# nicoloalbergoni/DeepLabV3Plus-Augmented-SuperResolution

Hardware: AMD Instinct MI355X
Metric: augmented-copies/sec (fwd+realign+SR-iter) @512x512 (higher is better)
Workload: dtype f32 (pointwise GEMMs: operands split into f16 hi+lo, hi*hi+hi*lo+lo*hi on f16 MFMA, f32 accumulate)

## Files before the change

### deeplabv3plus-augmented-superresolution_amd/csrc/sepconv.hip

```cpp
#include "asr_common.h"

#ifndef ASR_SEPCONV_PACKED_SPLIT
#define ASR_SEPCONV_PACKED_SPLIT 1
#endif

typedef float f32x4 __attribute__((ext_vector_type(4)));
typedef float f32x16 __attribute__((ext_vector_type(16)));
typedef _Float16 f16x4 __attribute__((ext_vector_type(4)));
typedef _Float16 f16x8 __attribute__((ext_vector_type(8)));

namespace {

constexpr int SF_TH = 8, SF_TW = 14, SF_VALID = SF_TH * SF_TW, SF_M = 128, SF_N = 128;

template <int CTRL>
__device__ __forceinline__ f32x4 sf_dpp4(f32x4 v) {
    f32x4 r;
#pragma unroll
    for (int i = 0; i < 4; ++i) {
        const float f = v[i];
        r[i] = __int_as_float(__builtin_amdgcn_mov_dpp(__float_as_int(f), CTRL, 0xF, 0xF, true));
    }
    return r;
}

__device__ __forceinline__ int sf_swz(int slot, int line) { return (slot & ~15) | ((slot ^ line) & 15); }

#ifdef ASR_DIAG_SEPCONV_MAX_VGPR
#define ASR_SEPCONV_ATTR __attribute__((amdgpu_num_vgpr(ASR_DIAG_SEPCONV_MAX_VGPR)))
#else
#define ASR_SEPCONV_ATTR
#endif
template <int CIN>
__global__ __launch_bounds__(512) ASR_PK_F32 ASR_SEPCONV_ATTR void sepconv_fused_kernel(const float* __restrict__ x, const float* __restrict__ wd,
                                                            const float* __restrict__ bd, const _Float16* __restrict__ wp,
                                                            const float* __restrict__ bp, float* __restrict__ y, int batch, int h,
                                                            int w, int ldx, int ldy, int npad, int pre_relu, int dw_relu,
                                                            int out_relu) {
#if ASR_SEPCONV_PACKED_SPLIT
    asr_enable_f16_saturation();
#endif
#ifdef ASR_DIAG_SEPCONV_TOP_VGPR
    ASR_DIAG_TOUCH_VGPR(ASR_DIAG_SEPCONV_TOP_VGPR);
#endif
    constexpr int QUADS = CIN / 4;
    constexpr int HALVES = 32 / QUADS;
    constexpr int RPT = SF_TH / HALVES;
    constexpr int LB = CIN * 4;
    constexpr int OCTS = CIN / 8;
    constexpr int A_BYTES = SF_M * LB, B_BYTES = OCTS * SF_N * 16;
    extern __shared__ __attribute__((aligned(16))) char sf_lds[];
    char* const A = sf_lds;
    char* const Bh = sf_lds + A_BYTES;
    char* const Bl = Bh + B_BYTES;
    const int tid = threadIdx.x, lane = tid & 63, wave = tid >> 6, l32 = lane & 31, hh = lane >> 5;
    typedef unsigned int u32x4 __attribute__((ext_vector_type(4)));
    {
        const long long plane = (long long)CIN * npad;
        for (int i = tid; i < OCTS * SF_N; i += 512) {
            const int oct = i >> 7, col = i & 127;
            const _Float16* src = wp + ((long long)oct * npad + col) * 8;
            *reinterpret_cast<u32x4*>(Bh + i * 16) = *reinterpret_cast<const u32x4*>(src);
            *reinterpret_cast<u32x4*>(Bl + i * 16) = *reinterpret_cast<const u32x4*>(src + plane);
        }
    }
    const int lane16 = lane & 15, slot = wave * 4 + (lane >> 4);
    const int q = slot % QUADS, ry0 = (slot / QUADS) * RPT, ch = q * 4;
    f32x4 wk[9];
#pragma unroll
    for (int t = 0; t < 9; ++t) wk[t] = *reinterpret_cast<const f32x4*>(wd + t * CIN + ch);
    const f32x4 bv = *reinterpret_cast<const f32x4*>(bd + ch);
    const f32x4 zero = {0.f, 0.f, 0.f, 0.f};
    const int wm = wave & 3, wn = wave >> 2;
    const float bp0 = bp[wn * 64 + l32], bp1 = bp[wn * 64 + 32 + l32];

    const int tiles_x = (w + SF_TW - 1) / SF_TW, tiles_y = (h + SF_TH - 1) / SF_TH;
    const long long total = (long long)batch * tiles_y * tiles_x;
    f32x4 in[RPT + 2];
    auto request_rows = [&](long long t) {
        const int tx0 = (int)(t % tiles_x) * SF_TW;
        const long long tt = t / tiles_x;
        const int ty0 = (int)(tt % tiles_y) * SF_TH;
        const float* xin = x + (tt / tiles_y) * h * w * ldx + ch;
        const int ixc = min(max(tx0 - 1 + lane16, 0), w - 1);
#pragma unroll
        for (int r = 0; r < RPT + 2; ++r) {
            const int iy = min(max(ty0 + ry0 - 1 + r, 0), h - 1);
            in[r] = *reinterpret_cast<const f32x4*>(xin + ((long long)iy * w + ixc) * ldx);
        }
    };
    const long long per_wg = (total + gridDim.x - 1) / gridDim.x;
    const long long first = (long long)blockIdx.x * per_wg, last = min(first + per_wg, total);
    if (first < last) request_rows(first);
    for (long long tile = first; tile < last; ++tile) {
        const int x0 = (int)(tile % tiles_x) * SF_TW;
        const long long tt = tile / tiles_x;
        const int y0 = (int)(tt % tiles_y) * SF_TH;
        const long long b = tt / tiles_y;
        __syncthreads();
        const int ix = x0 - 1 + lane16;
        const bool col_ok = ix >= 0 && ix < w;
        f32x4 win[3][3];
#pragma unroll
        for (int r = 0; r < RPT + 2; ++r) {
            const int iy = y0 + ry0 - 1 + r;
            f32x4 c = in[r];
            if (pre_relu) {
#pragma unroll
                for (int i = 0; i < 4; ++i) c[i] = fmaxf(c[i], 0.f);
            }
            c = (col_ok && iy >= 0 && iy < h) ? c : zero;
            win[2][1] = c;
            win[2][0] = sf_dpp4<0x111>(c);
            win[2][2] = sf_dpp4<0x101>(c);
            if (r >= 2) {
                f32x4 acc = bv;
#pragma unroll
                for (int ky = 0; ky < 3; ++ky)
#pragma unroll
                    for (int kx = 0; kx < 3; ++kx) acc += win[ky][kx] * wk[ky * 3 + kx];
                if (dw_relu) {
#pragma unroll
                    for (int i = 0; i < 4; ++i) acc[i] = fmaxf(acc[i], 0.f);
                }
                typedef unsigned int u32x2 __attribute__((ext_vector_type(2)));
#if ASR_SEPCONV_PACKED_SPLIT
                unsigned int h01, h23, l01, l23;
                asr_split4_f16_saturating_mode(acc[0], acc[1], acc[2], acc[3], h01, h23, l01, l23);
                u32x2 h2 = {h01, h23}, l2 = {l01, l23};
#else
                f16x4 hi, lo;
#pragma unroll
                for (int i = 0; i < 4; ++i) {
                    _Float16 hf, lf;
                    asr_split_f16(acc[i], hf, lf);
                    hi[i] = hf;
                    lo[i] = lf;
                }
                u32x2 h2 = __builtin_bit_cast(u32x2, hi), l2 = __builtin_bit_cast(u32x2, lo);
#endif
                {
                    const auto sx = __builtin_amdgcn_permlane16_swap(h2.x, l2.x, false, false);
                    const auto sy = __builtin_amdgcn_permlane16_swap(h2.y, l2.y, false, false);
                    h2.x = sx[0]; l2.x = sx[1];
                    h2.y = sy[0]; l2.y = sy[1];
                }
                const u32x4 out = {h2.x, h2.y, l2.x, l2.y};
                if (lane16 >= 1 && lane16 <= SF_TW) {
                    const int line = (ry0 + r - 2) * SF_TW + lane16 - 1;
                    *reinterpret_cast<u32x4*>(A + line * LB + sf_swz(((q & 1) ? OCTS : 0) + (q >> 1), line) * 16) = out;
                }
            }
#pragma unroll
            for (int k = 0; k < 3; ++k) {
                win[0][k] = win[1][k];
                win[1][k] = win[2][k];
            }
        }
        request_rows(min(tile + 1, last - 1));
        __syncthreads();
        f32x16 acc2[2];
#pragma unroll
        for (int j = 0; j < 2; ++j)
#pragma unroll
            for (int e = 0; e < 16; ++e) acc2[j][e] = 0.0f;
        const int m = wm * 32 + l32;
        const char* const aline = A + m * LB;
#pragma unroll
        for (int kk = 0; kk < CIN / 16; ++kk) {
            const int oct = 2 * kk + hh;
            const f16x8 ah = *reinterpret_cast<const f16x8*>(aline + sf_swz(oct, m) * 16);
            const f16x8 al = *reinterpret_cast<const f16x8*>(aline + sf_swz(OCTS + oct, m) * 16);
#pragma unroll
            for (int j = 0; j < 2; ++j) {
                const int col = wn * 64 + j * 32 + l32;
                const f16x8 bh = *reinterpret_cast<const f16x8*>(Bh + (oct * SF_N + col) * 16);
                const f16x8 bl = *reinterpret_cast<const f16x8*>(Bl + (oct * SF_N + col) * 16);
                acc2[j] = __builtin_amdgcn_mfma_f32_32x32x16_f16(al, bh, acc2[j], 0, 0, 0);
                acc2[j] = __builtin_amdgcn_mfma_f32_32x32x16_f16(ah, bl, acc2[j], 0, 0, 0);
                acc2[j] = __builtin_amdgcn_mfma_f32_32x32x16_f16(ah, bh, acc2[j], 0, 0, 0);
            }
        }
        float* const ybase = y + (b * h * w) * ldy + wn * 64 + l32;
#pragma unroll
        for (int e = 0; e < 16; ++e) {
            const int line = wm * 32 + (e & 3) + 8 * (e >> 2) + 4 * hh;
            const int ty = line / SF_TW, tx = line - ty * SF_TW;
            const int oy = y0 + ty, ox = x0 + tx;
            if (line < SF_VALID && oy < h && ox < w) {
                float* const o = ybase + ((long long)oy * w + ox) * ldy;
                float v0 = acc2[0][e] + bp0, v1 = acc2[1][e] + bp1;
                if (out_relu) { v0 = fmaxf(v0, 0.f); v1 = fmaxf(v1, 0.f); }
                o[0] = v0;
                o[32] = v1;
            }
        }
    }
}

template <int CIN>
int launch_sepconv_fused(const float* x, const float* wd, const float* bd, const void* wp, const float* bp, float* y, int batch,
                         int h, int w, int ldx, int ldy, int npad, int pre_relu, int dw_relu, int out_relu, hipStream_t s) {
    constexpr int lds = SF_M * CIN * 4 + 2 * (CIN / 8) * SF_N * 16;
    const int cus = asr_device_cu_count();
    ASR_REQUIRE(cus > 0, "asr_sepconv_fused_f16x3: cannot query the device");
    static AsrDeviceOnce once;
    ASR_HIP_CHECK(asr_allow_dynamic_lds(once, reinterpret_cast<const void*>(sepconv_fused_kernel<CIN>), lds));
    const long long tiles = (long long)batch * asr_cdiv(h, SF_TH) * asr_cdiv(w, SF_TW);
    const long long want = (long long)cus * (lds <= 80 * 1024 ? 2 : 1);
    const int grid = (int)(tiles < want ? tiles : want);
    hipLaunchKernelGGL(sepconv_fused_kernel<CIN>, dim3(grid), dim3(512), lds, s, x, wd, bd, reinterpret_cast<const _Float16*>(wp), bp, y,
                       batch, h, w, ldx, ldy, npad, pre_relu, dw_relu, out_relu);
    ASR_LAUNCH_CHECK();
    return ASR_OK;
}

}

extern "C" int asr_sepconv_fused_f16x3(const float* x, const float* w_dw, const float* bias_dw, const void* w_pw_packed,
                                       const float* bias_pw, float* y, int batch, int h, int w, int cin, int cout, int ldx,
                                       int ldy, int pre_relu, int dw_relu, int out_relu, asr_stream_t stream) {
    ASR_REQUIRE(x && w_dw && bias_dw && w_pw_packed && bias_pw && y, "asr_sepconv_fused_f16x3: null pointer");
    ASR_REQUIRE(batch > 0 && h > 0 && w > 0 && ldx >= cin && ldy >= cout, "asr_sepconv_fused_f16x3: bad geometry");
    ASR_UNSUPPORTED(!((cin == 64 || cin == 128) && cout == 128),
                    "asr_sepconv_fused_f16x3: cin in {64, 128} -> 128 only (got %d -> %d)", cin, cout);
    ASR_UNSUPPORTED((ldx & 3) || ((reinterpret_cast<uintptr_t>(x) | reinterpret_cast<uintptr_t>(w_dw) |
                                   reinterpret_cast<uintptr_t>(bias_dw) | reinterpret_cast<uintptr_t>(w_pw_packed)) & 15),
                    "asr_sepconv_fused_f16x3: ldx %% 4 == 0 and 16-byte aligned x / weights required");
    ASR_UNSUPPORTED((long long)h * w * ldx > 0x7fffffffLL, "asr_sepconv_fused_f16x3: image too large");
    hipStream_t s = asr_stream(stream);
    const int npad = 128;
    if (cin == 64)
        return launch_sepconv_fused<64>(x, w_dw, bias_dw, w_pw_packed, bias_pw, y, batch, h, w, ldx, ldy, npad, pre_relu, dw_relu, out_relu, s);
    return launch_sepconv_fused<128>(x, w_dw, bias_dw, w_pw_packed, bias_pw, y, batch, h, w, ldx, ldy, npad, pre_relu, dw_relu, out_relu, s);
}
```

Measured before the change: 2174.

## Walk vertical strips per workgroup and carry halo rows between steps

Result: no change. 2187, median of 6 (+0.6%).

```diff
diff --git a/deeplabv3plus-augmented-superresolution_amd/csrc/sepconv.hip b/deeplabv3plus-augmented-superresolution_amd/csrc/sepconv.hip
--- a/deeplabv3plus-augmented-superresolution_amd/csrc/sepconv.hip
+++ b/deeplabv3plus-augmented-superresolution_amd/csrc/sepconv.hip
@@ -53,6 +53,8 @@
     char* const A = sf_lds;
     char* const Bh = sf_lds + A_BYTES;
     char* const Bl = Bh + B_BYTES;
+    float* const bias2 = reinterpret_cast<float*>(A + SF_VALID * LB);
+    static_assert((SF_M - SF_VALID) * LB >= SF_N * 4, "the spare LDS lines hold the pointwise bias");
     const int tid = threadIdx.x, lane = tid & 63, wave = tid >> 6, l32 = lane & 31, hh = lane >> 5;
     typedef unsigned int u32x4 __attribute__((ext_vector_type(4)));
     {
@@ -72,38 +74,48 @@
     const f32x4 bv = *reinterpret_cast<const f32x4*>(bd + ch);
     const f32x4 zero = {0.f, 0.f, 0.f, 0.f};
     const int wm = wave & 3, wn = wave >> 2;
-    const float bp0 = bp[wn * 64 + l32], bp1 = bp[wn * 64 + 32 + l32];
-
-    const int tiles_x = (w + SF_TW - 1) / SF_TW, tiles_y = (h + SF_TH - 1) / SF_TH;
-    const long long total = (long long)batch * tiles_y * tiles_x;
+    if (tid < SF_N) bias2[tid] = bp[tid];
+
+    const int strips_x = (w + SF_TW - 1) / SF_TW;
+    const int steps = ((h + RPT - 1) / RPT + HALVES - 1) / HALVES;
+    const int hoff = HALVES > 1 ? steps * RPT : 0;
+    const int rbase = HALVES > 1 ? (ry0 ? hoff : 0) : 0;
+    const long long total = (long long)batch * strips_x * steps;
     f32x4 in[RPT + 2];
-    auto request_rows = [&](long long t) {
-        const int tx0 = (int)(t % tiles_x) * SF_TW;
-        const long long tt = t / tiles_x;
-        const int ty0 = (int)(tt % tiles_y) * SF_TH;
-        const float* xin = x + (tt / tiles_y) * h * w * ldx + ch;
-        const int ixc = min(max(tx0 - 1 + lane16, 0), w - 1);
-#pragma unroll
-        for (int r = 0; r < RPT + 2; ++r) {
-            const int iy = min(max(ty0 + ry0 - 1 + r, 0), h - 1);
+    auto request_rows = [&](long long b, int sx, int st, bool carry) {
+        const float* xin = x + b * h * w * ldx + ch;
+        const int ixc = min(max(sx * SF_TW - 1 + lane16, 0), w - 1);
+        const int yb = st * RPT + rbase - 1;
+        if (carry) {
+            in[0] = in[RPT];
+            in[1] = in[RPT + 1];
+        } else {
+#pragma unroll
+            for (int r = 0; r < 2; ++r) {
+                const int iy = min(max(yb + r, 0), h - 1);
+                in[r] = *reinterpret_cast<const f32x4*>(xin + ((long long)iy * w + ixc) * ldx);
+            }
+        }
+#pragma unroll
+        for (int r = 2; r < RPT + 2; ++r) {
+            const int iy = min(max(yb + r, 0), h - 1);
             in[r] = *reinterpret_cast<const f32x4*>(xin + ((long long)iy * w + ixc) * ldx);
         }
     };
     const long long per_wg = (total + gridDim.x - 1) / gridDim.x;
     const long long first = (long long)blockIdx.x * per_wg, last = min(first + per_wg, total);
-    if (first < last) request_rows(first);
-    for (long long tile = first; tile < last; ++tile) {
-        const int x0 = (int)(tile % tiles_x) * SF_TW;
-        const long long tt = tile / tiles_x;
-        const int y0 = (int)(tt % tiles_y) * SF_TH;
-        const long long b = tt / tiles_y;
+    int st = (int)(first % steps), sx = (int)((first / steps) % strips_x);
+    long long b = first / steps / strips_x;
+    if (first < last) request_rows(b, sx, st, false);
+    for (long long u = first; u < last; ++u) {
+        const int x0 = sx * SF_TW, y0 = st * RPT;
         __syncthreads();
         const int ix = x0 - 1 + lane16;
         const bool col_ok = ix >= 0 && ix < w;
         f32x4 win[3][3];
 #pragma unroll
         for (int r = 0; r < RPT + 2; ++r) {
-            const int iy = y0 + ry0 - 1 + r;
+            const int iy = y0 + rbase - 1 + r;
             f32x4 c = in[r];
             if (pre_relu) {
 #pragma unroll
@@ -157,7 +169,17 @@
                 win[1][k] = win[2][k];
             }
         }
-        request_rows(min(tile + 1, last - 1));
+        int nst = st + 1, nsx = sx;
+        long long nb = b;
+        if (nst == steps) {
+            nst = 0;
+            if (++nsx == strips_x) {
+                nsx = 0;
+                ++nb;
+            }
+        }
+        const bool more = u + 1 < last;
+        request_rows(more ? nb : b, more ? nsx : sx, more ? nst : st, more && nst != 0);
         __syncthreads();
         f32x16 acc2[2];
 #pragma unroll
@@ -181,12 +203,13 @@
                 acc2[j] = __builtin_amdgcn_mfma_f32_32x32x16_f16(ah, bh, acc2[j], 0, 0, 0);
             }
         }
+        const float bp0 = bias2[wn * 64 + l32], bp1 = bias2[wn * 64 + 32 + l32];
         float* const ybase = y + (b * h * w) * ldy + wn * 64 + l32;
 #pragma unroll
         for (int e = 0; e < 16; ++e) {
             const int line = wm * 32 + (e & 3) + 8 * (e >> 2) + 4 * hh;
             const int ty = line / SF_TW, tx = line - ty * SF_TW;
-            const int oy = y0 + ty, ox = x0 + tx;
+            const int oy = y0 + ty + (HALVES > 1 && ty >= RPT ? hoff - RPT : 0), ox = x0 + tx;
             if (line < SF_VALID && oy < h && ox < w) {
                 float* const o = ybase + ((long long)oy * w + ox) * ldy;
                 float v0 = acc2[0][e] + bp0, v1 = acc2[1][e] + bp1;
@@ -195,6 +218,9 @@
                 o[32] = v1;
             }
         }
+        b = nb;
+        sx = nsx;
+        st = nst;
     }
 }
 
```
